# facebookresearch/AudioDec

Hardware: AMD Instinct MI355X
Metric: 48 kHz hop-300 frames/s/GPU + per-frame encode+decode latency (ms) (higher is better)
Workload: dtype f32 (conv operands split into f16 hi + lo/2048 pairs, 3 f16 MFMAs per product sum, f32 accumulate)

## Files before the change

audiodec_amd/csrc/adk_common.h:

```cpp
#pragma once
#include <hip/hip_runtime.h>
#include <stdint.h>
#include <string>
#include <algorithm>
#include <cstring>
#include "../../include/audiodec_hip.h"

namespace adk {

void set_error(const std::string& msg);
int fail(int code, const std::string& msg);

#define ADK_HIP_CHECK(expr)                                                                   \
    do {                                                                                      \
        hipError_t _e = (expr);                                                               \
        if (_e != hipSuccess)                                                                 \
            return ::adk::fail(ADK_ERR_HIP, std::string(#expr) + ": " + hipGetErrorString(_e)); \
    } while (0)

struct ConvArgs {
    const float* in;   int in_rows, in_ch, in_row0, in_choff, in_gstride;
    float* out;        int out_rows, out_ch, out_cursor, out_choff;
    const float* res;  int res_rows, res_ch, res_cursor, res_choff, res_gstride;
    const float* w;    const float* wfrag;  const float* bias;
// ... 33 lines not shown
    float* out; int out_rows, out_cursor;
    int n, channels, batch, t;
};
int launch_ring_mean(const RingMeanArgs& m, hipStream_t s);
int launch_hist_replicate(float* ring, int rows, int channels, int cursor, int hist, int batch, hipStream_t s);
int launch_conv_direct(const ConvArgs& a, hipStream_t s);
bool conv_cin1_write_ok(const ConvArgs& a);
int launch_conv_cin1_write(const ConvArgs& a, const float* src, hipStream_t s);
struct Workspace { float* ptr = nullptr; size_t bytes = 0; size_t flags_offset = 0; unsigned epoch = 0;
                   int workgroups = 0; };
int launch_conv_mfma(const ConvArgs& a, hipStream_t s, Workspace& ws);
size_t conv_mfma_workspace_bytes(size_t* flags_offset);
bool conv_rl_supported(const ConvArgs& a);
bool conv_rl_preferred(const ConvArgs& a);
int launch_conv_rl(const ConvArgs& a, hipStream_t s);
bool conv_rl16_supported(const ConvArgs& a);
bool conv_rl16_preferred(const ConvArgs& a);
int launch_conv_rl16(const ConvArgs& a, hipStream_t s);
bool conv_rl16_fusable(const ConvArgs& a1, const ConvArgs& a2);
int launch_conv_rl16_fused(const ConvArgs& a1, const ConvArgs& a2, hipStream_t s);
bool conv_rb16_fusable(const ConvArgs* c, int n);
int launch_conv_rb16(const ConvArgs* c, int n, const int* keep, hipStream_t s);
const char* conv_rb16_name(const ConvArgs* c, int n);
bool conv_ou16_fusable(const ConvArgs& a1, const ConvArgs& a2);
int launch_conv_ou16(const ConvArgs& a1, const ConvArgs& a2, hipStream_t s);
bool conv_oc16_fusable(const ConvArgs& a1, const ConvArgs& a2);
int launch_conv_oc16(const ConvArgs& a1, const ConvArgs& a2, hipStream_t s);
bool conv_up16_supported(const ConvArgs& a);
int launch_conv_up16(const ConvArgs& a, hipStream_t s);
int launch_conv_sk16(const ConvArgs& a, hipStream_t s, Workspace& ws);
int conv_sk16_pick(const ConvArgs& a);
bool conv_gv16_preferred(const ConvArgs& a);
int conv_set_option(const char* name, int value);
int rvq_set_option(const char* name, int value);
int rvq_ema_set_option(const char* name, int value);
int launch_pack_split16(const float* w, float* out, int groups, int cout_g, int ktot, hipStream_t s);
int* flags_word();
inline int* conv_err_word(const ConvArgs& a) { return a.err ? a.err : flags_word(); }
constexpr int kMaxDevices = 64;
int flag_pool_acquire(int device, int** word);
void flag_pool_release(int device, int* word);
int flag_pool_fetch(int device, int* word, hipStream_t s, int* v);
int flag_pool_take(int device, int* word, int* v);
int flag_pool_fetch_all(int device, int* acc);
inline int current_device() { int d = 0; (void)hipGetDevice(&d); return (d >= 0 && d < kMaxDevices) ? d : 0; }
inline int device_of(const void* ptr) {
// ... 24 lines not shown
```

audiodec_amd/csrc/conv_rb16.hip:

```cpp
#include "adk_common.h"
#include <type_traits>
#include <cstdlib>

#ifndef ADK_RB16_PF32
#define ADK_RB16_PF32 2
#endif
#ifndef ADK_RB16_PF64
#define ADK_RB16_PF64 2
#endif
#ifndef ADK_RB16_PF128
#define ADK_RB16_PF128 3
#endif
#ifndef ADK_RB16_PIN_LOADS
#define ADK_RB16_PIN_LOADS 1
#endif
#ifndef ADK_RB16_ASYNC_TOUCH
#define ADK_RB16_ASYNC_TOUCH 1
#endif
#ifndef ADK_RB16_RING_SLOTS32
#define ADK_RB16_RING_SLOTS32 4
#endif
#ifndef ADK_RB16_HIST_LATE
#define ADK_RB16_HIST_LATE 1
#endif
#ifndef ADK_RB16_HIST_LATE128
// ... 32 lines not shown
constexpr int kRbMaxHist = 56;
constexpr int kRbTouchSink = 256;
constexpr float kRbLoScale = 2048.f, kRbLoInv = 1.f / 2048.f;

struct RbNode {
    float* base; int rows, ch, cursor, choff, gstride;
    int keep;
};
struct RbConv { const float* wfrag; const float* bias; int dil, hist, ksteps; unsigned w_bytes; };
struct RbArgs {
    RbNode node[kRbMaxConvs + 1];
    RbConv conv[kRbMaxConvs];
    int n_convs, batch, t, groups;
    int spw;
    int hm;
    int rps;
    int n_tiles;
    float slope; int* err;
    int warm;
    int n_main;
    int helpers;
    int helper_convs;
    int dbg_slot;
};

template <int ACT>
__device__ __forceinline__ float rb_act(float x, float slope) {
    if (ACT == ADK_ACT_ELU) return x > 0.f ? x : expm1_neg(x);
    if (ACT == ADK_ACT_LEAKY) return x > 0.f ? x : x * slope;
    return x;
}

__device__ __forceinline__ f16x8 rb_as_f16x8(const u32x4s& v) {
    union { u32x4s u; f16x8 h; } c; c.u = v; return c.h;
}

template <int C, int ACT>
__device__ __forceinline__ void rb_put8(unsigned char* dst, const float4& u, const float4& v, float slope) {
    const float x[8] = {u.x, u.y, u.z, u.w, v.x, v.y, v.z, v.w};
    f16x8 hi, lo;
#pragma unroll
    for (int j = 0; j < 8; ++j) {
        const float y = rb_act<ACT>(x[j], slope);
        const _Float16 h = (_Float16)y;
        hi[j] = h;
        lo[j] = (_Float16)((y - (float)h) * kRbLoScale);
// ... 78 lines not shown
        for (int sg = 0; sg < GS; ++sg) {
            const int s = i * GS + sg;
            const int tap = s / CH, ch = s - tap * CH;
            const int off = tap * dil_rs + 32 * ch;
            const f16x8 Ah = *reinterpret_cast<const f16x8*>(slot + (sg * MT + mt) * 2048);
            const f16x8 Al = *reinterpret_cast<const f16x8*>(slot + (sg * MT + mt) * 2048 + 1024);
            f16x8 bh[NA], bl[NA];
#pragma unroll
            for (int j = 0; j < NA; ++j) {
                bh[j] = *reinterpret_cast<const f16x8*>(x[j] + off);
                bl[j] = *reinterpret_cast<const f16x8*>(x[j] + off + 2 * C);
            }
#pragma unroll
            for (int j = 0; j < NA; ++j) m[j] = __builtin_amdgcn_mfma_f32_32x32x16_f16(Ah, bh[j], m[j], 0, 0, 0);
#pragma unroll
            for (int j = 0; j < NA; ++j) c[j] = __builtin_amdgcn_mfma_f32_32x32x16_f16(Ah, bl[j], c[j], 0, 0, 0);
#pragma unroll
            for (int j = 0; j < NA; ++j) c[j] = __builtin_amdgcn_mfma_f32_32x32x16_f16(Al, bh[j], c[j], 0, 0, 0);
        }
        rg.sl = rg.sl + 1 == WR ? 0 : rg.sl + 1;
    }
}

template <int C, int ACT, int TA, int TB, int NTW, int SMAX, int WPS, int PF, bool EARLY_RES, int LS, int WR>
__global__ __launch_bounds__(256, WPS) void conv_rb16_kernel(RbArgs r) {
    constexpr int RS = 4 * C + 16;
    constexpr int C8 = C / 8;
    constexpr int MT = C / 32;
    constexpr int NW = 4, NT = 64 * NW;
    constexpr int WM = NW / MT;
    constexpr bool BIAS_LDS = C < 128 && !(C == 64 && (SMAX == 2 || WR > 0));
    constexpr int RING_BYTES = WR * 4096;
    constexpr bool BIAS_LATE = WR > 0 && !BIAS_LDS;
    constexpr bool HIST_LATE = (((WR > 0 || ADK_RB16_HIST_LATE > 1) && WPS == 3) || (C == 128 && ADK_RB16_HIST_LATE128)) && ADK_RB16_HIST_LATE;
    constexpr int NHP = (SMAX * kRbMaxHist * C8 + NT - 1) / NT;
    extern __shared__ __attribute__((aligned(16))) unsigned char xs[];

    const int tid = threadIdx.x, lane = tid & 63;
    const int wave = __builtin_amdgcn_readfirstlane(tid >> 6);
    const int l31 = lane & 31, lh = lane >> 5;
    const unsigned lane16 = (unsigned)lane * 16u;
    if ((int)blockIdx.x >= r.n_main) {
        const int pad = (r.n_main + 7) & ~7;
        if (r.helpers <= 0 || (int)blockIdx.x < pad) return;
        const int h = (int)blockIdx.x - pad, xcd = h & 7, sub = h >> 3;
        typedef unsigned char __attribute__((address_space(3)))* lds_u8h_t;
        const unsigned sink = (unsigned)(size_t)(lds_u8h_t)xs;
        unsigned seen = 0;
        for (int i = xcd; i < r.n_main; i += 8) seen |= 1u << (i % r.groups);
        auto touch = [&](const unsigned char* ptr) __attribute__((always_inline)) {
            unsigned m0_keep_;
            asm volatile("s_mov_b32 %0, m0\n\ts_mov_b32 m0, %2\n\ts_nop 0\n\tglobal_load_lds_dword %1, off\n\ts_mov_b32 m0, %0"
                         : "=&s"(m0_keep_) : "v"(ptr), "s"(sink) : "memory");
        };
        for (int k = 0; k < r.helper_convs; ++k) {
            if (k == 1) {
                for (int i = xcd; i < r.n_main; i += 8) {
                    const int gi = i % r.groups, s0 = (i / r.groups) * r.spw, sc = min(r.spw, r.batch - s0);
// ... 57 lines not shown
        const int mt_ = MT == 1 ? 0 : q, sg_ = MT == 1 ? q : 0;
        return reinterpret_cast<const unsigned char*>(cv.wfrag) + ((size_t)((g * MT + mt_) * cv.ksteps + sg_)) * 2048u + (size_t)(wave & 1) * 1024u + lane16;
    };
    auto preload = [&](auto taps_c, const RbConv& cv) __attribute__((always_inline)) {
        constexpr int TAPS = decltype(taps_c)::value;
        if constexpr (WR > 0) {
            rb_ring_preload<C, TAPS, WR>(rg, ring_src(cv), wave);
        } else {
            constexpr int steps = TAPS * (C / 16);
            const __amdgpu_buffer_rsrc_t rs_ = __builtin_amdgcn_make_buffer_rsrc(const_cast<float*>(cv.wfrag), 0, cv.w_bytes, 0x00020000);
            const unsigned wb = (unsigned)((g * MT + mt) * cv.ksteps) * 2048u;
#pragma unroll
            for (int s = 0; s < PF; ++s) {
                if (s < steps) {
                    ah[s] = __builtin_amdgcn_raw_buffer_load_b128(rs_, lane16, wb + (unsigned)s * 2048u, 0);
                    al[s] = __builtin_amdgcn_raw_buffer_load_b128(rs_, lane16 + 1024u, wb + (unsigned)s * 2048u, 0);
                }
            }
        }
    };
    if constexpr (WR == 0) preload(std::integral_constant<int, TA>(), r.conv[0]);

    const unsigned touch_m0 = rg.lds_addr + (unsigned)RING_BYTES;
#if ADK_RB16_ASYNC_TOUCH
#define RB_TOUCH(ptr) do { unsigned m0_keep_; asm volatile("s_mov_b32 %0, m0\n\ts_mov_b32 m0, %2\n\ts_nop 0\n\tglobal_load_lds_dword %1, off\n\ts_mov_b32 m0, %0" \
                                                        : "=&s"(m0_keep_) : "v"(ptr), "s"(touch_m0) : "memory"); } while (0)
#else
#define RB_TOUCH(ptr) (void)*reinterpret_cast<const volatile unsigned*>(ptr)
#endif
    auto warm_weights = [&](const RbConv& cv) __attribute__((always_inline)) {
        const unsigned char* wbp = reinterpret_cast<const unsigned char*>(cv.wfrag) + (size_t)((g * MT + mt) * cv.ksteps) * 2048u;
        const int nlines = cv.ksteps * 16;
        const int ln = (int)__builtin_amdgcn_mbcnt_hi(~0u, __builtin_amdgcn_mbcnt_lo(~0u, 0u));
        for (int base_line = 64 * wi; base_line < nlines; base_line += 64 * WM) {
            const int line = min(base_line + ln, nlines - 1);
            RB_TOUCH(wbp + (size_t)line * 128u);
        }
    };
    if (r.warm) warm_weights(r.conv[0]);
    if constexpr (WR > 0) {
        if (r.warm) warm_weights(r.conv[1]);
    }
    for (int k = 1; k < (r.warm ? r.n_convs : 0); ++k) {
        const RbNode& nd = r.node[k];
        const int hk = r.conv[k].hist;
        constexpr int LPR = (C * 4 + 127) / 128;
        const int total = scur * hk * LPR;
        for (int i = tid; i < total; i += NT) {
            const int s = i / (hk * LPR), rem_ = i - s * hk * LPR;
            const int rr = rem_ / LPR, li = rem_ - rr * LPR;
            int row = nd.cursor - hk + rr;
            if (row < 0) row += nd.rows;
            RB_TOUCH(nd.base + ((size_t)(b0 + s) * nd.rows + row) * nd.ch + nd.choff + g * nd.gstride + 32 * li);
        }
    }
    if constexpr (WR > 0) preload(std::integral_constant<int, TA>(), r.conv[0]);

    {
        const RbNode& nd = r.node[0];
        const int h0 = r.conv[0].hist;
        const int per = (h0 + T) * C8;
        const int total = scur * per;
        constexpr int SB = 4;
        for (int i0 = tid; i0 < total; i0 += SB * NT) {
            float4 u[SB], v[SB]; int dst[SB];
#pragma unroll
            for (int k = 0; k < SB; ++k) {
                const int i = i0 + k * NT;
                dst[k] = -1;
                if (i < total) {
                    const int s = i / per, rem_ = i - s * per;
                    const int rr = rem_ / C8, c8 = rem_ - rr * C8;
                    int row = nd.cursor - h0 + rr;
                    if (row < 0) row += nd.rows;
                    if (row >= nd.rows) row -= nd.rows;
                    const float4* p = reinterpret_cast<const float4*>(nd.base + ((size_t)(b0 + s) * nd.rows + row) * nd.ch + nd.choff + g * nd.gstride + 8 * c8);
                    u[k] = p[0]; v[k] = p[1];
                    dst[k] = (s * r.rps + r.hm - h0 + rr) * RS + 16 * c8;
                }
            }
#pragma unroll
            for (int k = 0; k < SB; ++k)
                if (dst[k] >= 0) rb_put8<C, ACT>(xs + dst[k], u[k], v[k], r.slope);
        }
        if constexpr (BIAS_LDS) {
            for (int i = tid; i < r.n_convs * C; i += NT) {
                const int k = i / C, c = i - k * C;
                bias_lds[i] = r.conv[k].bias ? r.conv[k].bias[g * C + c] : 0.f;
            }
        }
    }
    __syncthreads();
    RB_STAMP(1);

    bool bad = false;

    auto hist_issue = [&](int k, float4 (&hu)[NHP], float4 (&hv)[NHP]) __attribute__((always_inline)) {
        const RbNode& nd = r.node[k];
        const int hk = r.conv[k].hist;
        const int per = hk * C8, total = scur * per;
#pragma unroll
        for (int q = 0; q < NHP; ++q) {
            const int i = tid + q * NT;
            hu[q] = hv[q] = make_float4(0.f, 0.f, 0.f, 0.f);
            if (i < total) {
                const int s = i / per, rem_ = i - s * per;
                const int rr = rem_ / C8, c8 = rem_ - rr * C8;
                int row = nd.cursor - hk + rr;
                if (row < 0) row += nd.rows;
                const float4* p = reinterpret_cast<const float4*>(nd.base + ((size_t)(b0 + s) * nd.rows + row) * nd.ch + nd.choff + g * nd.gstride + 8 * c8);
                hu[q] = p[0]; hv[q] = p[1];
            }
        }
    };
    auto hist_commit = [&](int k, const float4 (&hu)[NHP], const float4 (&hv)[NHP]) __attribute__((always_inline)) {
        const int hk = r.conv[k].hist;
        const int per = hk * C8, total = scur * per;
#pragma unroll
        for (int q = 0; q < NHP; ++q) {
            const int i = tid + q * NT;
            if (i < total) {
                const int s = i / per, rem_ = i - s * per;
                const int rr = rem_ / C8, c8 = rem_ - rr * C8;
                rb_put8<C, ACT>(xs + (s * r.rps + r.hm - hk + rr) * RS + 16 * c8, hu[q], hv[q], r.slope);
            }
        }
    };
    auto bias_issue = [&](int k, float4 (&breg)[4]) __attribute__((always_inline)) {
#pragma unroll
        for (int qd = 0; qd < 4; ++qd) {
            breg[qd] = make_float4(0.f, 0.f, 0.f, 0.f);
            if constexpr (!BIAS_LDS) {
                if (r.conv[k].bias) breg[qd] = *reinterpret_cast<const float4*>(r.conv[k].bias + g * C + mt * 32 + 8 * qd + 4 * lh);
            }
        }
    };
    auto finish = [&](int k, bool vld, const f32x16& am, const f32x16& ac, const float4 (&breg)[4], float (&h)[16]) __attribute__((always_inline)) {
        const bool hb = r.conv[k].bias != nullptr;
#pragma unroll
        for (int qd = 0; qd < 4; ++qd) {
            float4 bb = breg[qd];
            if constexpr (BIAS_LDS) bb = *reinterpret_cast<const float4*>(bias_lds + k * C + mt * 32 + 8 * qd + 4 * lh);
            float v0 = fmaf(ac[4 * qd], kRbLoInv, am[4 * qd]), v1 = fmaf(ac[4 * qd + 1], kRbLoInv, am[4 * qd + 1]);
            float v2 = fmaf(ac[4 * qd + 2], kRbLoInv, am[4 * qd + 2]), v3 = fmaf(ac[4 * qd + 3], kRbLoInv, am[4 * qd + 3]);
            bad |= vld & (!(fabsf(v0) <= 3.0e38f) | !(fabsf(v1) <= 3.0e38f) | !(fabsf(v2) <= 3.0e38f) | !(fabsf(v3) <= 3.0e38f));
            if (hb) { v0 += bb.x; v1 += bb.y; v2 += bb.z; v3 += bb.w; }
            h[4 * qd] = v0; h[4 * qd + 1] = v1; h[4 * qd + 2] = v2; h[4 * qd + 3] = v3;
        }
    };
    auto ring_store = [&](int k, int j, const float (&h)[16], bool all) __attribute__((always_inline)) {
        const RbNode& nd = r.node[k];
        if (!valid[j] || !(all || tj[j] >= T - nd.keep)) return;
        int row = nd.cursor + tj[j];
        if (row >= nd.rows) row -= nd.rows;
        float* p = nd.base + ((size_t)(b0 + sj[j]) * nd.rows + row) * nd.ch + nd.choff + g * nd.gstride + mt * 32 + 4 * lh;
#pragma unroll
        for (int qd = 0; qd < 4; ++qd)
            *reinterpret_cast<float4*>(p + 8 * qd) = make_float4(h[4 * qd], h[4 * qd + 1], h[4 * qd + 2], h[4 * qd + 3]);
    };
    auto res_load = [&](int k, int j, float4 (&rr)[4]) __attribute__((always_inline)) {
        const RbNode& nd = r.node[k];
        int row = nd.cursor + tj[j];
        if (row >= nd.rows) row -= nd.rows;
        const float* p = nd.base + ((size_t)(b0 + sj[j]) * nd.rows + row) * nd.ch + nd.choff + g * nd.gstride + mt * 32 + 4 * lh;
#pragma unroll
        for (int qd = 0; qd < 4; ++qd) {
            const f32x4 v = __builtin_nontemporal_load(reinterpret_cast<const f32x4*>(p + 8 * qd));
            rr[qd] = make_float4(v[0], v[1], v[2], v[3]);
        }
    };
    auto lds_put = [&](int j, const float (&h)[16]) __attribute__((always_inline)) {
        if (!valid[j]) return;
        unsigned char* row = xs + lrow[j] * RS;
#pragma unroll
        for (int qd = 0; qd < 4; ++qd) {
            const int ml = mt * 32 + 8 * qd + 4 * lh;
            f16x4 hi, lo;
#pragma unroll
            for (int e = 0; e < 4; ++e) {
                const float y = rb_act<ACT>(h[4 * qd + e], r.slope);
                const _Float16 hh = (_Float16)y;
                hi[e] = hh;
                lo[e] = (_Float16)((y - (float)hh) * kRbLoScale);
            }
            *reinterpret_cast<f16x4*>(row + 2 * ml) = hi;
            *reinterpret_cast<f16x4*>(row + 2 * C + 2 * ml) = lo;
        }
    };
    auto conv_loop = [&](auto taps_c, const RbConv& cv, f32x16 (&m)[NTW], f32x16 (&c)[NTW]) __attribute__((always_inline)) {
        constexpr int TAPS = decltype(taps_c)::value;
        const unsigned char* x[NTW];
#pragma unroll
// ... 10 lines not shown
        }
    };

    const int units = r.n_convs >> 1;
#pragma unroll 1
    for (int u = 0; u < units; ++u) {
        {
            const int k = 2 * u;
            const RbConv cv = r.conv[k];
            f32x16 m[NTW], c[NTW];
#pragma unroll
            for (int j = 0; j < NTW; ++j)
#pragma unroll
                for (int e = 0; e < 16; ++e) { m[j][e] = 0.f; c[j][e] = 0.f; }
            float4 breg[4];
            if constexpr (!BIAS_LATE) bias_issue(k, breg);
            if (WR == 0 && r.warm) warm_weights(r.conv[k + 1]);
            conv_loop(std::integral_constant<int, TA>(), cv, m, c);
            RB_STAMP(2 + 4 * k);
            if constexpr (BIAS_LATE) bias_issue(k, breg);
            if (WR > 0 && r.warm && k + 2 < r.n_convs) warm_weights(r.conv[k + 2]);
            preload(std::integral_constant<int, TB>(), r.conv[k + 1]);
            float4 hu[NHP], hv[NHP];
            if constexpr (!HIST_LATE) hist_issue(k + 1, hu, hv);
            float h[NTW][16];
#pragma unroll
            for (int j = 0; j < NTW; ++j) { finish(k, valid[j], m[j], c[j], breg, h[j]); ring_store(k + 1, j, h[j], false); }
            if constexpr (HIST_LATE) { __builtin_amdgcn_sched_barrier(0); hist_issue(k + 1, hu, hv); }
            RB_STAMP(3 + 4 * k);
            __syncthreads();
            RB_STAMP(4 + 4 * k);
#pragma unroll
            for (int j = 0; j < NTW; ++j) lds_put(j, h[j]);
            hist_commit(k + 1, hu, hv);
            __syncthreads();
            RB_STAMP(5 + 4 * k);
        }
        {
            const int k = 2 * u + 1;
            const RbConv cv = r.conv[k];
            const bool last = u + 1 == units;
            const int kn = last ? k : k + 1;
            f32x16 m[NTW], c[NTW];
#pragma unroll
            for (int j = 0; j < NTW; ++j)
#pragma unroll
                for (int e = 0; e < 16; ++e) { m[j][e] = 0.f; c[j][e] = 0.f; }
            float4 breg[4];
            if constexpr (!BIAS_LATE) bias_issue(k, breg);
            if (WR == 0 && !last && r.warm) warm_weights(r.conv[kn]);
            float4 rr[NTW][4];
            if constexpr (EARLY_RES) {
#pragma unroll
                for (int j = 0; j < NTW; ++j) res_load(k - 1, j, rr[j]);
            }
            conv_loop(std::integral_constant<int, TB>(), cv, m, c);
            RB_STAMP(2 + 4 * k);
            if constexpr (BIAS_LATE) bias_issue(k, breg);
            if constexpr (WR > 0) {
                if (!last) {
                    if (r.warm && k + 2 < r.n_convs) warm_weights(r.conv[k + 2]);
                    preload(std::integral_constant<int, TA>(), r.conv[kn]);
                }
            } else {
                preload(std::integral_constant<int, TA>(), r.conv[kn]);
            }
            float4 hu[NHP], hv[NHP];
            if constexpr (!HIST_LATE) hist_issue(kn, hu, hv);
            if constexpr (!EARLY_RES) {
#pragma unroll
                for (int j = 0; j < NTW; ++j) res_load(k - 1, j, rr[j]);
            }
            float h[NTW][16];
#pragma unroll
            for (int j = 0; j < NTW; ++j) {
                finish(k, valid[j], m[j], c[j], breg, h[j]);
#pragma unroll
                for (int qd = 0; qd < 4; ++qd) { h[j][4 * qd] += rr[j][qd].x; h[j][4 * qd + 1] += rr[j][qd].y; h[j][4 * qd + 2] += rr[j][qd].z; h[j][4 * qd + 3] += rr[j][qd].w; }
                ring_store(k + 1, j, h[j], true);
            }
            if constexpr (HIST_LATE) { __builtin_amdgcn_sched_barrier(0); hist_issue(kn, hu, hv); }
            RB_STAMP(3 + 4 * k);
            if (!last) {
                __syncthreads();
                RB_STAMP(4 + 4 * k);
#pragma unroll
                for (int j = 0; j < NTW; ++j) lds_put(j, h[j]);
                hist_commit(kn, hu, hv);
                __syncthreads();
                RB_STAMP(5 + 4 * k);
            }
        }
    }
    if (bad) atomicOr(r.err, 8);
}

struct RbPlan { int C, ta, tb, ntw, spw, n_tiles, hm, rps, wr; size_t lds; long long blocks; };

int rb_knob(const char* name, int dflt) { const char* e = getenv(name); return e ? atoi(e) : dflt; }

int rb_streams_per_wg(int C, int batch, int t, int groups) {
    static const int env128 = rb_knob("ADK_RB16_SPW", 0);
    static const int env64 = rb_knob("ADK_RB16_SPW64", 0);
    int s = (C == 128) ? 2 : 1;
    if (env128 > 0 && C == 128) s = env128;
    if (env64 > 0 && C == 64) s = env64;
    const int wm = 4 / (C / 32);
    const int max_ntw = C == 128 ? 2 : 4;
    while (s > 1 && (s > batch || (s * t + 31) / 32 > max_ntw * wm)) --s;
    static const int few = rb_knob("ADK_RB16_FEW128", 128);
    if (C == 128 && s == 2 && env128 <= 0 && (long long)batch * groups <= few && t <= 32) s = 1;
    return s;
}

int rb_ring_slots(int C, int ntw, int spw, long long blocks) {
    static const int on = rb_knob("ADK_RB16_RING", 1);
    if (!on || (blocks <= 128 && on < 3)) return 0;
    if (C == 32 && ntw == 2) return 3;
    if (C == 32 && ntw == 3 && on >= 2) return ADK_RB16_RING_SLOTS32;
    if (C == 64 && ntw == 2 && spw == 1) return 3;
    return 0;
}

bool rb_plan(const ConvArgs* c, int n, RbPlan& pl) {
    const ConvArgs& a0 = c[0];
    pl.C = a0.cin_g; pl.ta = a0.taps; pl.tb = c[1].taps;
    const int T = a0.t_out;
    const int wm = 4 / (pl.C / 32);
    pl.spw = rb_streams_per_wg(pl.C, a0.batch, T, a0.groups);
    pl.n_tiles = (pl.spw * T + 31) / 32;
    pl.ntw = std::max(pl.C == 128 ? 1 : 2, (pl.n_tiles + wm - 1) / wm);
    if (pl.ntw > 4 || (pl.C == 128 && pl.ntw > 2)) return false;
    pl.hm = 0;
    for (int k = 0; k < n; ++k) pl.hm = std::max(pl.hm, (c[k].taps - 1) * c[k].dilation);
    if (pl.hm > kRbMaxHist) return false;
    pl.rps = pl.hm + T;
    pl.wr = rb_ring_slots(pl.C, pl.ntw, pl.spw, (long long)((a0.batch + pl.spw - 1) / pl.spw) * a0.groups);
    const bool bias_lds = pl.C < 128 && !(pl.C == 64 && (pl.spw > 1 || pl.ntw > 2 || pl.wr > 0));
    pl.lds = (size_t)pl.spw * pl.rps * (4 * pl.C + 16) + (bias_lds ? (size_t)n * pl.C * 4 : 0) + (size_t)pl.wr * 4096 + kRbTouchSink;
    if (pl.lds > 160 * 1024 || pl.spw > (pl.C == 128 ? 2 : (pl.C == 64 ? 2 : 1))) return false;
    pl.blocks = (long long)((a0.batch + pl.spw - 1) / pl.spw) * a0.groups;
    return pl.blocks <= 0x7fffffffLL;
}

bool aligned16(const void* p) { return (reinterpret_cast<uintptr_t>(p) & 15) == 0; }

}

bool conv_rb16_fusable(const ConvArgs* c, int n) {
    if (n < 2 || n > kRbMaxConvs || (n & 1)) return false;
    const ConvArgs& a0 = c[0];
    const int C = a0.cin_g;
    if (C != 32 && C != 64 && C != 128) return false;
    if (a0.act_in != ADK_ACT_ELU && a0.act_in != ADK_ACT_LEAKY) return false;
    const int ta = a0.taps, tb = c[1].taps;
    if (!((ta == 11 && tb == 11) || (ta == 7 && tb == 7) || (ta == 3 && tb == 3) || (ta == 7 && tb == 1))) return false;
    if (a0.act_in == ADK_ACT_ELU && !(ta == 7 && tb == 1)) return false;
    if (a0.act_in == ADK_ACT_LEAKY && tb == 1) return false;
    if (a0.t_out < 1 || a0.batch < 1) return false;
    for (int k = 0; k < n; ++k) {
        const ConvArgs& a = c[k];
        const bool isB = k & 1;
        if (!a.wfrag || !aligned16(a.wfrag) || (a.bias && !aligned16(a.bias))) return false;
        if (a.cin_g != C || a.cout_g != C || a.groups != a0.groups || a.stride != 1 || a.up != 1 || a.cout_real != a.groups * C) return false;
        if (a.taps != (isB ? tb : ta) || a.dilation < 1) return false;
        if (a.act_in != a0.act_in || a.slope != a0.slope || a.act_out != ADK_ACT_NONE) return false;
        if (a.batch != a0.batch || a.t_out != a0.t_out) return false;
        if ((a.in_ch % 4) || (a.in_choff % 4) || (a.in_gstride % 4) || (a.out_ch % 4) || (a.out_choff % 4) || !aligned16(a.in) || !aligned16(a.out)) return false;
        if (a.in_rows < a.t_out + (a.taps - 1) * a.dilation || a.out_rows < a.t_out) return false;
        if (k > 0) {
            const ConvArgs& p = c[k - 1];
            if (a.in != p.out || a.in_rows != p.out_rows || a.in_ch != p.out_ch || a.in_choff != p.out_choff || a.in_gstride != C) return false;
            if ((a.in_row0 + (a.taps - 1) * a.dilation) % a.in_rows != p.out_cursor) return false;
        }
        if (!isB) {
            if (a.res) return false;
        } else {
            const ConvArgs& f = c[k - 1];
            if (!a.res || a.res != f.in || a.res_rows != f.in_rows || a.res_ch != f.in_ch || a.res_choff != f.in_choff || a.res_gstride != f.in_gstride) return false;
            if (a.res_cursor != (f.in_row0 + (f.taps - 1) * f.dilation) % f.in_rows) return false;
        }
    }
    RbPlan pl;
    return rb_plan(c, n, pl);
}

namespace {
template <int C, int ACT, int TA, int TB, int NTW, int SMAX, int WPS, int PF, bool EARLY_RES, int LS, int WR>
int rb_go(const RbArgs& r, const RbPlan& pl, hipStream_t s) {
    auto kern = conv_rb16_kernel<C, ACT, TA, TB, NTW, SMAX, WPS, PF, EARLY_RES, LS, WR>;
    if (pl.lds > 64 * 1024) {
        static bool attr_set_dev[kMaxDevices] = {};
        bool& attr_set = attr_set_dev[current_device()];
        if (!attr_set) {
            ADK_HIP_CHECK(hipFuncSetAttribute(reinterpret_cast<const void*>(kern), hipFuncAttributeMaxDynamicSharedMemorySize, 160 * 1024));
            attr_set = true;
        }
    }
    const unsigned grid = r.helpers > 0 ? (unsigned)(((r.n_main + 7) & ~7) + 8 * r.helpers) : (unsigned)pl.blocks;
    hipLaunchKernelGGL(kern, dim3(grid), dim3(256), pl.lds, s, r);
    ADK_HIP_CHECK(hipGetLastError());
    return ADK_OK;
}

template <int C, int NTW, int SMAX, int WPS, int PF, bool EARLY_RES, int LS, int WR = 0>
int rb_by_taps(const RbArgs& r, const RbPlan& pl, int act, hipStream_t s) {
    if (act == ADK_ACT_ELU) return rb_go<C, ADK_ACT_ELU, 7, 1, NTW, SMAX, WPS, PF, EARLY_RES, LS, WR>(r, pl, s);
    if (pl.ta == 11) return rb_go<C, ADK_ACT_LEAKY, 11, 11, NTW, SMAX, WPS, PF, EARLY_RES, LS, WR>(r, pl, s);
    if (pl.ta == 7) return rb_go<C, ADK_ACT_LEAKY, 7, 7, NTW, SMAX, WPS, PF, EARLY_RES, LS, WR>(r, pl, s);
    return rb_go<C, ADK_ACT_LEAKY, 3, 3, NTW, SMAX, WPS, PF, EARLY_RES, LS, WR>(r, pl, s);
}
}

int launch_conv_rb16(const ConvArgs* c, int n, const int* keep, hipStream_t s) {
    if (!conv_rb16_fusable(c, n)) return ADK_ERR_STATE;
    RbPlan pl;
    if (!rb_plan(c, n, pl)) return ADK_ERR_STATE;
    if (c[0].n_total == 0) return ADK_OK;
    RbArgs r;
    memset(&r, 0, sizeof(r));
    const ConvArgs& a0 = c[0];
    r.node[0].base = const_cast<float*>(a0.in); r.node[0].rows = a0.in_rows; r.node[0].ch = a0.in_ch;
    r.node[0].cursor = (a0.in_row0 + (a0.taps - 1) * a0.dilation) % a0.in_rows;
    r.node[0].choff = a0.in_choff; r.node[0].gstride = a0.in_gstride; r.node[0].keep = 0;
    for (int k = 0; k < n; ++k) {
        const ConvArgs& a = c[k];
        RbNode& nd = r.node[k + 1];
        nd.base = a.out; nd.rows = a.out_rows; nd.ch = a.out_ch; nd.cursor = a.out_cursor; nd.choff = a.out_choff; nd.gstride = a.cout_g;
        nd.keep = k + 1 < n ? std::max(keep[k], (c[k + 1].taps - 1) * c[k + 1].dilation) : 0;
        RbConv& cv = r.conv[k];
        cv.wfrag = a.wfrag; cv.bias = a.bias; cv.dil = a.dilation; cv.hist = (a.taps - 1) * a.dilation;
        cv.ksteps = (a.ktot + 63) / 64 * 4;
        cv.w_bytes = (unsigned)((unsigned long long)a.groups * (a.cout_g / 32) * cv.ksteps * 2048ull);
    }
    r.n_convs = n; r.batch = a0.batch; r.t = a0.t_out; r.groups = a0.groups;
    r.spw = pl.spw; r.hm = pl.hm; r.rps = pl.rps; r.n_tiles = pl.n_tiles;
    r.slope = a0.slope; r.err = conv_err_word(a0);
    static const int warm_env = rb_knob("ADK_RB16_WARM", -1);
    r.warm = warm_env == 2 ? (pl.C <= 64) : (warm_env >= 0 ? warm_env : (pl.C <= 64 && pl.blocks <= 384 && pl.blocks > 128));
#if ADK_RB16_DBG & 1
    r.dbg_slot = g_rb_launch++;
#endif
    {
        static const int per_xcd = rb_knob("ADK_RB16_HELPERS", 4);
        static const int max_blocks = rb_knob("ADK_RB16_HELPER_BLOCKS", 64);
        constexpr long long kHelperBytes = 3584 * 1024;
        r.n_main = (int)pl.blocks; r.helpers = 0; r.helper_convs = 0;
        if (per_xcd > 0 && pl.blocks <= max_blocks && a0.groups <= 32) {
            int worst = 0;
            for (int x = 0; x < 8; ++x) {
                unsigned seen = 0; int cnt = 0;
                for (long long i = x; i < pl.blocks; i += 8) { const unsigned bit = 1u << (int)(i % a0.groups); if (!(seen & bit)) { seen |= bit; ++cnt; } }
                worst = std::max(worst, cnt);
            }
            long long bytes = 0;
            int kc = 0;
            for (; kc < n; ++kc) {
                const long long one = (long long)(pl.C / 32) * r.conv[kc].ksteps * 2048ll * worst;
                if (bytes + one > kHelperBytes) break;
                bytes += one;
            }
            if (kc > 0 && worst > 0) { r.helpers = per_xcd; r.helper_convs = kc; }
        }
    }
    const int act = a0.act_in;
    if (pl.C == 32 && pl.wr > 0) {
        if (pl.ntw == 2) return rb_by_taps<32, 2, 1, 3, 1, true, 0, 3>(r, pl, act, s);
        if (pl.ta == 11) return rb_by_taps<32, 3, 1, 2, 1, false, 0, ADK_RB16_RING_SLOTS32>(r, pl, act, s);
        return rb_by_taps<32, 3, 1, 2, 1, true, 0, ADK_RB16_RING_SLOTS32>(r, pl, act, s);
    }
    if (pl.C == 64 && pl.wr > 0) return rb_by_taps<64, 2, 1, 3, 1, ADK_RB16_EARLY64, 0, 3>(r, pl, act, s);
    const bool few = pl.blocks <= 128;
    if (pl.C == 32) {
        if (pl.ntw == 2 && few) return rb_by_taps<32, 2, 1, 2, ADK_RB16_PF32, true, 0>(r, pl, act, s);
        if (pl.ntw == 2) return rb_by_taps<32, 2, 1, 3, ADK_RB16_PF32, true, 0>(r, pl, act, s);
        if (pl.ntw == 3 && pl.ta == 11) return rb_by_taps<32, 3, 1, 2, ADK_RB16_PF32, false, 0>(r, pl, act, s);
        if (pl.ntw == 3) return rb_by_taps<32, 3, 1, 2, ADK_RB16_PF32, true, 0>(r, pl, act, s);
        return rb_by_taps<32, 4, 1, 2, 2, false, 0>(r, pl, act, s);
    }
    if (pl.C == 64) {
        if (pl.ntw == 2 && pl.spw == 1 && few) return rb_by_taps<64, 2, 1, 2, ADK_RB16_PF64, true, 0>(r, pl, act, s);
        if (pl.ntw == 2 && pl.spw == 1) return rb_by_taps<64, 2, 1, 3, ADK_RB16_PF64, true, 0>(r, pl, act, s);
        if (pl.ntw <= 3) return rb_by_taps<64, 3, 2, 2, 2, true, 0>(r, pl, act, s);
        return rb_by_taps<64, 4, 2, 2, 2, false, 0>(r, pl, act, s);
    }
    if (pl.ntw == 1) return rb_by_taps<128, 1, 1, 2, ADK_RB16_PF128, true, 4>(r, pl, act, s);
    return rb_by_taps<128, 2, 2, 2, ADK_RB16_PF128, true, 4>(r, pl, act, s);
}

const char* conv_rb16_name(const ConvArgs* c, int n) {
    (void)n;
    return c[0].cin_g == 32 ? "conv_rb16<32>" : (c[0].cin_g == 64 ? "conv_rb16<64>" : "conv_rb16<128>");
}

}
```

audiodec_amd/csrc/program.hip:

```cpp
#include "adk_common.h"
#include <vector>
#include <cstring>
#include <cstdio>
#include <cstdlib>
#include <mutex>
#include <atomic>

namespace adk {

static thread_local std::string g_err;
void set_error(const std::string& msg) { g_err = msg; }
int fail(int code, const std::string& msg) { g_err = msg; return code; }

static int build_args(const adk_conv_desc& d, const adk_ring_view& in, const adk_ring_view& out,
                      const adk_ring_view& res, int batch, int t_out, ConvArgs& a) {
    if ((!d.w && !d.w_frag) || !in.base || !out.base) return fail(ADK_ERR_ARG, "conv: null weight/in/out pointer");
    if (d.cin_g <= 0 || d.cout_g <= 0 || d.groups <= 0 || d.taps <= 0 || d.stride <= 0 || d.dilation <= 0 ||
        d.up <= 0 || d.cout_real <= 0 || d.hist < 0)
        return fail(ADK_ERR_SHAPE, "conv: non-positive geometry");
    if (batch < 0 || t_out < 0) return fail(ADK_ERR_SHAPE, "conv: negative batch / t_out");
    if ((long long)batch * t_out > 0x7fffffffLL) return fail(ADK_ERR_SHAPE, "conv: batch * t_out overflows");
    const long long M = (long long)d.groups * d.cout_g;
    if (M != (long long)d.up * d.cout_real) return fail(ADK_ERR_SHAPE, "conv: groups*cout_g != up*cout_real");
    if (d.up > 1 && d.groups != 1) return fail(ADK_ERR_SHAPE, "conv: transposed form needs groups == 1");
// ... 115 lines not shown
    const bool rl = mf && ((impl == ADK_IMPL_MFMA_ROWS && conv_rl_supported(a)) || (impl == ADK_IMPL_AUTO && g_use_rl && conv_rl_preferred(a)));
    if (rl) return a.cin_g == 32 ? "conv_rl<32>" : "conv_rl<64>";
    if (mf) return conv_mfma_cfg_name(conv_mfma_pick(a));
    return a.groups * a.cout_g == 1 ? "conv_cout1" : (a.cin_g == 1 && a.taps == 7 ? "conv_cin1" : "conv_direct");
}

}

using namespace adk;

extern "C" const char* adk_last_error(void) { return g_err.c_str(); }
extern "C" int adk_abi_version(void) { return ADK_ABI_VERSION; }
extern "C" int adk_set_conv_cfg(int32_t cfg) { conv_mfma_force_cfg(cfg); return ADK_OK; }
extern "C" int adk_set_option(const char* name, int32_t value) {
    if (!name) return fail(ADK_ERR_ARG, "adk_set_option: null name");
    read_env();
    if (!strcmp(name, "chain_max_channels")) { g_chain_max_c = value < 0 ? 0 : value; return ADK_OK; }
    if (!strcmp(name, "chain_min_channels")) { g_chain_min_c = value < 0 ? 0 : value; return ADK_OK; }
    if (!strcmp(name, "chain_min_blocks")) { g_chain_min_blocks = value < 0 ? 0 : value; return ADK_OK; }
    if (!strcmp(name, "conv_ou16")) { g_use_ou = value != 0; return ADK_OK; }
    if (!strcmp(name, "conv_oc16")) { g_use_oc = value != 0; return ADK_OK; }
    if (!strcmp(name, "conv_cin1w")) { g_use_cw = value != 0; return ADK_OK; }
    if (conv_set_option(name, value) == 0) return ADK_OK;
    {
        const int r = rvq_set_option(name, value);
        if (r == 0) return ADK_OK;
        if (r < 0) return fail(ADK_ERR_ARG, std::string("adk_set_option: bad value for ") + name);
    }
    {
        const int r = rvq_ema_set_option(name, value);
        if (r == 0) return ADK_OK;
        if (r < 0) return fail(ADK_ERR_ARG, std::string("adk_set_option: bad value for ") + name);
    }
    return fail(ADK_ERR_ARG, std::string("adk_set_option: unknown option ") + name);
}

extern "C" int adk_streamk_plan(int64_t tiles, int32_t chunks, int32_t cap, int32_t* plan) {
    if (!plan || tiles < 1 || tiles >= (1ll << 31) / 64 || chunks < 1 || chunks > (1 << 20) || cap < 0) return fail(ADK_ERR_ARG, "adk_streamk_plan: bad argument");
    int out[4];
    const int rc = streamk_plan(tiles, chunks, cap, out);
    for (int i = 0; i < 4; ++i) plan[i] = out[i];
    return rc;
}

extern "C" int64_t adk_streamk_range_start(int64_t tiles, int32_t chunks, const int32_t* plan, int32_t r) {
    if (!plan || tiles < 1 || chunks < 1 || plan[0] < 1 || r < 0 || r > plan[0]) return -1;
// ... 676 lines not shown
```

Measured before the change: 291,800.

## Stage residual-block history rows and residuals in LDS for the fused rb16 chain

```diff
diff --git a/audiodec_amd/csrc/adk_common.h b/audiodec_amd/csrc/adk_common.h
--- a/audiodec_amd/csrc/adk_common.h
+++ b/audiodec_amd/csrc/adk_common.h
@@ -79,6 +79,7 @@
 bool conv_rb16_fusable(const ConvArgs* c, int n);
 int launch_conv_rb16(const ConvArgs* c, int n, const int* keep, hipStream_t s);
 const char* conv_rb16_name(const ConvArgs* c, int n);
+int conv_rb16_set_option(const char* name, int value);
 bool conv_ou16_fusable(const ConvArgs& a1, const ConvArgs& a2);
 int launch_conv_ou16(const ConvArgs& a1, const ConvArgs& a2, hipStream_t s);
 bool conv_oc16_fusable(const ConvArgs& a1, const ConvArgs& a2);
diff --git a/audiodec_amd/csrc/conv_rb16.hip b/audiodec_amd/csrc/conv_rb16.hip
--- a/audiodec_amd/csrc/conv_rb16.hip
+++ b/audiodec_amd/csrc/conv_rb16.hip
@@ -1,6 +1,8 @@
 #include "adk_common.h"
 #include <type_traits>
 #include <cstdlib>
+#include <atomic>
+#include <mutex>
 
 #ifndef ADK_RB16_PF32
 #define ADK_RB16_PF32 2
@@ -79,6 +81,9 @@
     int helpers;
     int helper_convs;
     int dbg_slot;
+    int side_rows;
+    int side_off[kRbMaxConvs];
+    int res_lds;
 };
 
 template <int ACT>
@@ -203,7 +208,7 @@
     }
 }
 
-template <int C, int ACT, int TA, int TB, int NTW, int SMAX, int WPS, int PF, bool EARLY_RES, int LS, int WR>
+template <int C, int ACT, int TA, int TB, int NTW, int SMAX, int WPS, int PF, bool EARLY_RES, int LS, int WR, bool ON_CHIP = false>
 __global__ __launch_bounds__(256, WPS) void conv_rb16_kernel(RbArgs r) {
     constexpr int RS = 4 * C + 16;
     constexpr int C8 = C / 8;
@@ -214,7 +219,9 @@
     constexpr int RING_BYTES = WR * 4096;
     constexpr bool BIAS_LATE = WR > 0 && !BIAS_LDS;
     constexpr bool HIST_LATE = (((WR > 0 || ADK_RB16_HIST_LATE > 1) && WPS == 3) || (C == 128 && ADK_RB16_HIST_LATE128)) && ADK_RB16_HIST_LATE;
-    constexpr int NHP = (SMAX * kRbMaxHist * C8 + NT - 1) / NT;
+    constexpr int NHP = ON_CHIP ? 1 : (SMAX * kRbMaxHist * C8 + NT - 1) / NT;
+    static_assert(!ON_CHIP || SMAX <= 2, "the side-area copy tells the streams of a workgroup apart by one compare");
+    constexpr bool RES_LDS = ON_CHIP && C < 128;
     extern __shared__ __attribute__((aligned(16))) unsigned char xs[];
 
     const int tid = threadIdx.x, lane = tid & 63;
@@ -318,6 +325,8 @@
     if constexpr (WR == 0) preload(std::integral_constant<int, TA>(), r.conv[0]);
 
     const unsigned touch_m0 = rg.lds_addr + (unsigned)RING_BYTES;
+    const int side_base = (int)ring_off + RING_BYTES + kRbTouchSink;
+    const int res_base = side_base + r.spw * r.side_rows * RS;
 #if ADK_RB16_ASYNC_TOUCH
 #define RB_TOUCH(ptr) do { unsigned m0_keep_; asm volatile("s_mov_b32 %0, m0\n\ts_mov_b32 m0, %2\n\ts_nop 0\n\tglobal_load_lds_dword %1, off\n\ts_mov_b32 m0, %0" \
                                                         : "=&s"(m0_keep_) : "v"(ptr), "s"(touch_m0) : "memory"); } while (0)
@@ -337,7 +346,7 @@
     if constexpr (WR > 0) {
         if (r.warm) warm_weights(r.conv[1]);
     }
-    for (int k = 1; k < (r.warm ? r.n_convs : 0); ++k) {
+    for (int k = 1; k < ((r.warm && !ON_CHIP) ? r.n_convs : 0); ++k) {
         const RbNode& nd = r.node[k];
         const int hk = r.conv[k].hist;
         constexpr int LPR = (C * 4 + 127) / 128;
@@ -352,32 +361,88 @@
     }
     if constexpr (WR > 0) preload(std::integral_constant<int, TA>(), r.conv[0]);
 
+    auto res_load = [&](int k, int j, float4 (&rr)[4]) __attribute__((always_inline)) {
+        const RbNode& nd = r.node[k];
+        int row = nd.cursor + tj[j];
+        if (row >= nd.rows) row -= nd.rows;
+        const float* p = nd.base + ((size_t)(b0 + sj[j]) * nd.rows + row) * nd.ch + nd.choff + g * nd.gstride + mt * 32 + 4 * lh;
+#pragma unroll
+        for (int qd = 0; qd < 4; ++qd) {
+            const f32x4 v = __builtin_nontemporal_load(reinterpret_cast<const f32x4*>(p + 8 * qd));
+            rr[qd] = make_float4(v[0], v[1], v[2], v[3]);
+        }
+    };
+    static_assert(!RES_LDS || SMAX == 1, "one stream per workgroup: residual row t sits hm + t = lrow rows behind res_base - hm rows, the address lds_put computes anyway");
+    const int res_off = res_base - r.hm * RS;
+    auto res_put = [&](int j, const float4 (&v)[4]) __attribute__((always_inline)) {
+        if (!valid[j]) return;
+        unsigned char* p = xs + lrow[j] * RS + res_off + 4 * (mt * 32 + 4 * lh);
+#pragma unroll
+        for (int qd = 0; qd < 4; ++qd) *reinterpret_cast<float4*>(p + 32 * qd) = v[qd];
+    };
+    auto res_get = [&](int j, float4 (&v)[4]) __attribute__((always_inline)) {
+        const unsigned char* p = xs + lrow[j] * RS + res_off + 4 * (mt * 32 + 4 * lh);
+#pragma unroll
+        for (int qd = 0; qd < 4; ++qd) v[qd] = *reinterpret_cast<const float4*>(p + 32 * qd);
+    };
+    float4 rr[NTW][4];
+    if constexpr (ON_CHIP) {
+        if (!RES_LDS || r.res_lds) {
+#pragma unroll
+            for (int j = 0; j < NTW; ++j) res_load(0, j, rr[j]);
+        }
+    }
+
     {
         const RbNode& nd = r.node[0];
         const int h0 = r.conv[0].hist;
         const int per = (h0 + T) * C8;
-        const int total = scur * per;
-        constexpr int SB = 4;
+        const int total0 = scur * per;
+        const int per_side = ON_CHIP ? r.side_rows * C8 : 0;
+        const int total = total0 + scur * per_side;
+        constexpr int SB = (ON_CHIP && WPS < 3) ? 8 : 4;
         for (int i0 = tid; i0 < total; i0 += SB * NT) {
             float4 u[SB], v[SB]; int dst[SB];
 #pragma unroll
             for (int k = 0; k < SB; ++k) {
                 const int i = i0 + k * NT;
                 dst[k] = -1;
+                const bool side = ON_CHIP && i >= total0;
+                const int q = side ? i - total0 : i, pp = side ? per_side : per;
+                const int s = q / pp, rem_ = q - s * pp;
+                const int rr = rem_ / C8, c8 = rem_ - rr * C8;
+                int row = nd.cursor - h0 + rr;
+                if (row < 0) row += nd.rows;
+                if (row >= nd.rows) row -= nd.rows;
+                const float* p = nd.base + ((size_t)(b0 + s) * nd.rows + row) * nd.ch + nd.choff + g * nd.gstride + 8 * c8;
+                int d = (s * r.rps + r.hm - h0 + rr) * RS + 16 * c8;
+                if constexpr (ON_CHIP) {
+                    constexpr int K0 = TB == 1 ? 2 : 1;
+#pragma unroll
+                    for (int kk = K0; kk < kRbMaxConvs; kk += K0) {
+                        const RbNode& nk = r.node[kk];
+                        const int hk = r.conv[kk].hist, lr = rr - r.side_off[kk];
+                        int rk = nk.cursor - hk + lr;
+                        if (rk < 0) rk += nk.rows;
+                        const float* pk = nk.base + ((size_t)(b0 + s) * nk.rows + rk) * nk.ch + nk.choff + g * nk.gstride + 8 * c8;
+                        if (side && lr >= 0 && lr < hk) p = pk;
+                    }
+                    if (side) d = side_base + (s * r.side_rows + rr) * RS + 16 * c8;
+                }
                 if (i < total) {
-                    const int s = i / per, rem_ = i - s * per;
-                    const int rr = rem_ / C8, c8 = rem_ - rr * C8;
-                    int row = nd.cursor - h0 + rr;
-                    if (row < 0) row += nd.rows;
-                    if (row >= nd.rows) row -= nd.rows;
-                    const float4* p = reinterpret_cast<const float4*>(nd.base + ((size_t)(b0 + s) * nd.rows + row) * nd.ch + nd.choff + g * nd.gstride + 8 * c8);
-                    u[k] = p[0]; v[k] = p[1];
-                    dst[k] = (s * r.rps + r.hm - h0 + rr) * RS + 16 * c8;
+                    u[k] = reinterpret_cast<const float4*>(p)[0]; v[k] = reinterpret_cast<const float4*>(p)[1];
+                    dst[k] = d;
                 }
             }
 #pragma unroll
             for (int k = 0; k < SB; ++k)
                 if (dst[k] >= 0) rb_put8<C, ACT>(xs + dst[k], u[k], v[k], r.slope);
+        }
+        if constexpr (RES_LDS) {
+            if (r.res_lds) {
+#pragma unroll
+                for (int j = 0; j < NTW; ++j) res_put(j, rr[j]);
+            }
         }
         if constexpr (BIAS_LDS) {
             for (int i = tid; i < r.n_convs * C; i += NT) {
@@ -422,6 +487,27 @@
             }
         }
     };
+    auto hist_copy = [&](int k) __attribute__((always_inline)) {
+        constexpr int PR = C / 4;
+        const int hk = r.conv[k].hist;
+        const int per = hk * PR, total = scur * per;
+        const unsigned char* src = xs + side_base + r.side_off[k] * RS;
+        unsigned char* dst = xs + (r.hm - hk) * RS;
+        constexpr int UB = 4;
+        for (int i0 = tid; i0 < total; i0 += UB * NT) {
+            u32x4s v[UB]; int d[UB];
+#pragma unroll
+            for (int q = 0; q < UB; ++q) {
+                const int i = min(i0 + q * NT, total - 1);
+                const int s = (SMAX > 1 && i >= per) ? 1 : 0, rem_ = i - s * per;
+                const int rw = rem_ / PR, pc = rem_ - rw * PR;
+                v[q] = *reinterpret_cast<const u32x4s*>(src + (s * r.side_rows + rw) * RS + 16 * pc);
+                d[q] = (s * r.rps + rw) * RS + 16 * pc;
+            }
+#pragma unroll
+            for (int q = 0; q < UB; ++q) *reinterpret_cast<u32x4s*>(dst + d[q]) = v[q];
+        }
+    };
     auto bias_issue = [&](int k, float4 (&breg)[4]) __attribute__((always_inline)) {
 #pragma unroll
         for (int qd = 0; qd < 4; ++qd) {
@@ -453,17 +539,6 @@
 #pragma unroll
         for (int qd = 0; qd < 4; ++qd)
             *reinterpret_cast<float4*>(p + 8 * qd) = make_float4(h[4 * qd], h[4 * qd + 1], h[4 * qd + 2], h[4 * qd + 3]);
-    };
-    auto res_load = [&](int k, int j, float4 (&rr)[4]) __attribute__((always_inline)) {
-        const RbNode& nd = r.node[k];
-        int row = nd.cursor + tj[j];
-        if (row >= nd.rows) row -= nd.rows;
-        const float* p = nd.base + ((size_t)(b0 + sj[j]) * nd.rows + row) * nd.ch + nd.choff + g * nd.gstride + mt * 32 + 4 * lh;
-#pragma unroll
-        for (int qd = 0; qd < 4; ++qd) {
-            const f32x4 v = __builtin_nontemporal_load(reinterpret_cast<const f32x4*>(p + 8 * qd));
-            rr[qd] = make_float4(v[0], v[1], v[2], v[3]);
-        }
     };
     auto lds_put = [&](int j, const float (&h)[16]) __attribute__((always_inline)) {
         if (!valid[j]) return;
@@ -520,17 +595,17 @@
             if (WR > 0 && r.warm && k + 2 < r.n_convs) warm_weights(r.conv[k + 2]);
             preload(std::integral_constant<int, TB>(), r.conv[k + 1]);
             float4 hu[NHP], hv[NHP];
-            if constexpr (!HIST_LATE) hist_issue(k + 1, hu, hv);
+            if constexpr (!HIST_LATE && !ON_CHIP) hist_issue(k + 1, hu, hv);
             float h[NTW][16];
 #pragma unroll
             for (int j = 0; j < NTW; ++j) { finish(k, valid[j], m[j], c[j], breg, h[j]); ring_store(k + 1, j, h[j], false); }
-            if constexpr (HIST_LATE) { __builtin_amdgcn_sched_barrier(0); hist_issue(k + 1, hu, hv); }
+            if constexpr (HIST_LATE && !ON_CHIP) { __builtin_amdgcn_sched_barrier(0); hist_issue(k + 1, hu, hv); }
             RB_STAMP(3 + 4 * k);
             __syncthreads();
             RB_STAMP(4 + 4 * k);
 #pragma unroll
             for (int j = 0; j < NTW; ++j) lds_put(j, h[j]);
-            hist_commit(k + 1, hu, hv);
+            if constexpr (ON_CHIP) hist_copy(k + 1); else hist_commit(k + 1, hu, hv);
             __syncthreads();
             RB_STAMP(5 + 4 * k);
         }
@@ -547,8 +622,7 @@
             float4 breg[4];
             if constexpr (!BIAS_LATE) bias_issue(k, breg);
             if (WR == 0 && !last && r.warm) warm_weights(r.conv[kn]);
-            float4 rr[NTW][4];
-            if constexpr (EARLY_RES) {
+            if constexpr (EARLY_RES && !ON_CHIP) {
 #pragma unroll
                 for (int j = 0; j < NTW; ++j) res_load(k - 1, j, rr[j]);
             }
@@ -564,27 +638,33 @@
                 preload(std::integral_constant<int, TA>(), r.conv[kn]);
             }
             float4 hu[NHP], hv[NHP];
-            if constexpr (!HIST_LATE) hist_issue(kn, hu, hv);
-            if constexpr (!EARLY_RES) {
+            if constexpr (!HIST_LATE && !ON_CHIP) hist_issue(kn, hu, hv);
+            if constexpr (!EARLY_RES && !ON_CHIP) {
 #pragma unroll
                 for (int j = 0; j < NTW; ++j) res_load(k - 1, j, rr[j]);
             }
             float h[NTW][16];
 #pragma unroll
             for (int j = 0; j < NTW; ++j) {
+                if constexpr (RES_LDS) { if (r.res_lds) res_get(j, rr[j]); else res_load(k - 1, j, rr[j]); }
                 finish(k, valid[j], m[j], c[j], breg, h[j]);
 #pragma unroll
                 for (int qd = 0; qd < 4; ++qd) { h[j][4 * qd] += rr[j][qd].x; h[j][4 * qd + 1] += rr[j][qd].y; h[j][4 * qd + 2] += rr[j][qd].z; h[j][4 * qd + 3] += rr[j][qd].w; }
                 ring_store(k + 1, j, h[j], true);
-            }
-            if constexpr (HIST_LATE) { __builtin_amdgcn_sched_barrier(0); hist_issue(kn, hu, hv); }
+                if constexpr (ON_CHIP) {
+#pragma unroll
+                    for (int qd = 0; qd < 4; ++qd) rr[j][qd] = make_float4(h[j][4 * qd], h[j][4 * qd + 1], h[j][4 * qd + 2], h[j][4 * qd + 3]);
+                    if constexpr (RES_LDS) { if (!last && r.res_lds) res_put(j, rr[j]); }
+                }
+            }
+            if constexpr (HIST_LATE && !ON_CHIP) { __builtin_amdgcn_sched_barrier(0); hist_issue(kn, hu, hv); }
             RB_STAMP(3 + 4 * k);
             if (!last) {
                 __syncthreads();
                 RB_STAMP(4 + 4 * k);
 #pragma unroll
                 for (int j = 0; j < NTW; ++j) lds_put(j, h[j]);
-                hist_commit(kn, hu, hv);
+                if constexpr (ON_CHIP) hist_copy(kn); else hist_commit(kn, hu, hv);
                 __syncthreads();
                 RB_STAMP(5 + 4 * k);
             }
@@ -593,7 +673,7 @@
     if (bad) atomicOr(r.err, 8);
 }
 
-struct RbPlan { int C, ta, tb, ntw, spw, n_tiles, hm, rps, wr; size_t lds; long long blocks; };
+struct RbPlan { int C, ta, tb, ntw, spw, n_tiles, hm, rps, wr; size_t lds; long long blocks; int onchip, side_rows, res_lds; };
 
 int rb_knob(const char* name, int dflt) { const char* e = getenv(name); return e ? atoi(e) : dflt; }
 
@@ -618,6 +698,12 @@
     if (C == 32 && ntw == 3 && on >= 2) return ADK_RB16_RING_SLOTS32;
     if (C == 64 && ntw == 2 && spw == 1) return 3;
     return 0;
+}
+
+std::atomic<int> g_rb_onchip{1};
+std::once_flag g_rb_onchip_once;
+void rb_onchip_read_env() {
+    std::call_once(g_rb_onchip_once, [] { const char* e = getenv("ADK_RB16_ONCHIP"); if (e) g_rb_onchip.store(atoi(e) != 0); });
 }
 
 bool rb_plan(const ConvArgs* c, int n, RbPlan& pl) {
@@ -638,7 +724,20 @@
     pl.lds = (size_t)pl.spw * pl.rps * (4 * pl.C + 16) + (bias_lds ? (size_t)n * pl.C * 4 : 0) + (size_t)pl.wr * 4096 + kRbTouchSink;
     if (pl.lds > 160 * 1024 || pl.spw > (pl.C == 128 ? 2 : (pl.C == 64 ? 2 : 1))) return false;
     pl.blocks = (long long)((a0.batch + pl.spw - 1) / pl.spw) * a0.groups;
-    return pl.blocks <= 0x7fffffffLL;
+    if (pl.blocks > 0x7fffffffLL) return false;
+    pl.onchip = 0; pl.side_rows = 0; pl.res_lds = 0;
+    rb_onchip_read_env();
+    static const int oc_blocks = rb_knob("ADK_RB16_ONCHIP_BLOCKS", 128);
+    static const int oc_mask = rb_knob("ADK_RB16_ONCHIP_MASK", 7);
+    static const int oc_res = rb_knob("ADK_RB16_ONCHIP_RES", 1);
+    const bool inst = (pl.C == 128) || (pl.C == 64 && pl.ntw == 2 && pl.spw == 1 && (pl.wr > 0 || pl.blocks <= 128)) || (pl.C == 32 && pl.ntw == 3 && pl.wr == 0);
+    if (g_rb_onchip.load() && a0.act_in == ADK_ACT_ELU && pl.ta == 7 && pl.tb == 1 && pl.blocks <= std::min(oc_blocks, 256) && (oc_mask & (pl.C / 32)) && inst) {
+        int side = 0;
+        for (int k = 1; k < n; ++k) side += (c[k].taps - 1) * c[k].dilation;
+        const size_t lds = pl.lds + (size_t)pl.spw * (side + ((pl.C < 128 && oc_res) ? T : 0)) * (4 * pl.C + 16);
+        if (side > 0 && lds <= 160 * 1024) { pl.onchip = 1; pl.side_rows = side; pl.lds = lds; pl.res_lds = pl.C < 128 && oc_res; }
+    }
+    return true;
 }
 
 bool aligned16(const void* p) { return (reinterpret_cast<uintptr_t>(p) & 15) == 0; }
@@ -684,9 +783,9 @@
 }
 
 namespace {
-template <int C, int ACT, int TA, int TB, int NTW, int SMAX, int WPS, int PF, bool EARLY_RES, int LS, int WR>
+template <int C, int ACT, int TA, int TB, int NTW, int SMAX, int WPS, int PF, bool EARLY_RES, int LS, int WR, bool ON_CHIP = false>
 int rb_go(const RbArgs& r, const RbPlan& pl, hipStream_t s) {
-    auto kern = conv_rb16_kernel<C, ACT, TA, TB, NTW, SMAX, WPS, PF, EARLY_RES, LS, WR>;
+    auto kern = conv_rb16_kernel<C, ACT, TA, TB, NTW, SMAX, WPS, PF, EARLY_RES, LS, WR, ON_CHIP>;
     if (pl.lds > 64 * 1024) {
         static bool attr_set_dev[kMaxDevices] = {};
         bool& attr_set = attr_set_dev[current_device()];
@@ -701,8 +800,12 @@
     return ADK_OK;
 }
 
-template <int C, int NTW, int SMAX, int WPS, int PF, bool EARLY_RES, int LS, int WR = 0>
+template <int C, int NTW, int SMAX, int WPS, int PF, bool EARLY_RES, int LS, int WR = 0, bool OC = false>
 int rb_by_taps(const RbArgs& r, const RbPlan& pl, int act, hipStream_t s) {
+    if (pl.onchip) {
+        if constexpr (OC) { if (act == ADK_ACT_ELU) return rb_go<C, ADK_ACT_ELU, 7, 1, NTW, SMAX, WPS, PF, EARLY_RES, LS, WR, true>(r, pl, s); }
+        return ADK_ERR_STATE;
+    }
     if (act == ADK_ACT_ELU) return rb_go<C, ADK_ACT_ELU, 7, 1, NTW, SMAX, WPS, PF, EARLY_RES, LS, WR>(r, pl, s);
     if (pl.ta == 11) return rb_go<C, ADK_ACT_LEAKY, 11, 11, NTW, SMAX, WPS, PF, EARLY_RES, LS, WR>(r, pl, s);
     if (pl.ta == 7) return rb_go<C, ADK_ACT_LEAKY, 7, 7, NTW, SMAX, WPS, PF, EARLY_RES, LS, WR>(r, pl, s);
@@ -734,6 +837,8 @@
     r.n_convs = n; r.batch = a0.batch; r.t = a0.t_out; r.groups = a0.groups;
     r.spw = pl.spw; r.hm = pl.hm; r.rps = pl.rps; r.n_tiles = pl.n_tiles;
     r.slope = a0.slope; r.err = conv_err_word(a0);
+    r.side_rows = pl.side_rows; r.res_lds = pl.res_lds;
+    for (int k = 1, off = 0; k < n && pl.onchip; ++k) { r.side_off[k] = off; off += r.conv[k].hist; }
     static const int warm_env = rb_knob("ADK_RB16_WARM", -1);
     r.warm = warm_env == 2 ? (pl.C <= 64) : (warm_env >= 0 ? warm_env : (pl.C <= 64 && pl.blocks <= 384 && pl.blocks > 128));
 #if ADK_RB16_DBG & 1
@@ -767,23 +872,31 @@
         if (pl.ta == 11) return rb_by_taps<32, 3, 1, 2, 1, false, 0, ADK_RB16_RING_SLOTS32>(r, pl, act, s);
         return rb_by_taps<32, 3, 1, 2, 1, true, 0, ADK_RB16_RING_SLOTS32>(r, pl, act, s);
     }
-    if (pl.C == 64 && pl.wr > 0) return rb_by_taps<64, 2, 1, 3, 1, ADK_RB16_EARLY64, 0, 3>(r, pl, act, s);
+    if (pl.C == 64 && pl.wr > 0) return rb_by_taps<64, 2, 1, 3, 1, ADK_RB16_EARLY64, 0, 3, true>(r, pl, act, s);
     const bool few = pl.blocks <= 128;
     if (pl.C == 32) {
         if (pl.ntw == 2 && few) return rb_by_taps<32, 2, 1, 2, ADK_RB16_PF32, true, 0>(r, pl, act, s);
         if (pl.ntw == 2) return rb_by_taps<32, 2, 1, 3, ADK_RB16_PF32, true, 0>(r, pl, act, s);
         if (pl.ntw == 3 && pl.ta == 11) return rb_by_taps<32, 3, 1, 2, ADK_RB16_PF32, false, 0>(r, pl, act, s);
-        if (pl.ntw == 3) return rb_by_taps<32, 3, 1, 2, ADK_RB16_PF32, true, 0>(r, pl, act, s);
+        if (pl.ntw == 3) return rb_by_taps<32, 3, 1, 2, ADK_RB16_PF32, true, 0, 0, true>(r, pl, act, s);
         return rb_by_taps<32, 4, 1, 2, 2, false, 0>(r, pl, act, s);
     }
     if (pl.C == 64) {
-        if (pl.ntw == 2 && pl.spw == 1 && few) return rb_by_taps<64, 2, 1, 2, ADK_RB16_PF64, true, 0>(r, pl, act, s);
+        if (pl.ntw == 2 && pl.spw == 1 && few) return rb_by_taps<64, 2, 1, 2, ADK_RB16_PF64, true, 0, 0, true>(r, pl, act, s);
         if (pl.ntw == 2 && pl.spw == 1) return rb_by_taps<64, 2, 1, 3, ADK_RB16_PF64, true, 0>(r, pl, act, s);
         if (pl.ntw <= 3) return rb_by_taps<64, 3, 2, 2, 2, true, 0>(r, pl, act, s);
         return rb_by_taps<64, 4, 2, 2, 2, false, 0>(r, pl, act, s);
     }
-    if (pl.ntw == 1) return rb_by_taps<128, 1, 1, 2, ADK_RB16_PF128, true, 4>(r, pl, act, s);
-    return rb_by_taps<128, 2, 2, 2, ADK_RB16_PF128, true, 4>(r, pl, act, s);
+    if (pl.ntw == 1) return rb_by_taps<128, 1, 1, 2, ADK_RB16_PF128, true, 4, 0, true>(r, pl, act, s);
+    return rb_by_taps<128, 2, 2, 2, ADK_RB16_PF128, true, 4, 0, true>(r, pl, act, s);
+}
+
+int conv_rb16_set_option(const char* name, int value) {
+    if (strcmp(name, "chain_onchip")) return 1;
+    if (value != 0 && value != 1) return -1;
+    rb_onchip_read_env();
+    g_rb_onchip.store(value);
+    return 0;
 }
 
 const char* conv_rb16_name(const ConvArgs* c, int n) {
diff --git a/audiodec_amd/csrc/program.hip b/audiodec_amd/csrc/program.hip
--- a/audiodec_amd/csrc/program.hip
+++ b/audiodec_amd/csrc/program.hip
@@ -161,6 +161,11 @@
     if (!strcmp(name, "conv_oc16")) { g_use_oc = value != 0; return ADK_OK; }
     if (!strcmp(name, "conv_cin1w")) { g_use_cw = value != 0; return ADK_OK; }
     if (conv_set_option(name, value) == 0) return ADK_OK;
+    {
+        const int r = conv_rb16_set_option(name, value);
+        if (r == 0) return ADK_OK;
+        if (r < 0) return fail(ADK_ERR_ARG, std::string("adk_set_option: bad value for ") + name);
+    }
     {
         const int r = rvq_set_option(name, value);
         if (r == 0) return ADK_OK;
```

Result: slower. 282,500 (-3.2%).
